# joaobuibergen/roms-trunk-mgh

Hardware: AMD Instinct MI355X
Metric: simulated-days/wall-sec (higher is better)
Workload: dtype f64; 1 GPU; BENCHMARK3 2048x256x30 NT=2 nonlinear 3-D step incl. 59 step2d calls, U3/C4 tracer advection, analytic atmospheric forcing, bulk fluxes + KPP + diagnostics every step; tiling=1x1, halo_transport=none, rccl_ranks=0, graph_exchanges=1, ndtfast=20, finite=True

## Files before the change

### roms_trunk_mgh_amd/csrc/k_diag.hip

```cpp
#include "roms_dev.h"

int roms_entry_check(const char *name);

namespace {

__global__ void __launch_bounds__(BLK_X *BLK_Y)
k_wvelocity(const RomsDev *__restrict__ c, int ninp)
{
  DEV_PROLOGUE(c)
  const Blk XB = xcd_block();
  const int i = b.Istr + XB.x * BLK_X + threadIdx.x;
  const int j = b.Jstr + XB.y * BLK_Y + threadIdx.y;
  if (i > b.Iend || j > b.Jend) return;
  const long a = I2(i, j);
  const gcd_t u = (gcd_t)(c->F.u + (long)(ninp - 1) * n3r), v = (gcd_t)(c->F.v + (long)(ninp - 1) * n3r);
  const gcd_t z_r = (gcd_t)c->F.z_r, z_w = (gcd_t)c->F.z_w, W = (gcd_t)c->F.W;
  const gd_t wvel = (gd_t)c->F.wvel;
  const gcd_t pm = (gcd_t)c->F.pm, pn = (gcd_t)c->F.pn;
  const double pmw = pm[a - 1] + pm[a], pme = pm[a] + pm[a + 1];
  const double pns = pn[a - ni] + pn[a], pnn = pn[a] + pn[a + ni];
  const double pmn = pm[a] * pn[a];
  auto vert_at = [&](int k) {
    const long q = a + (long)(k - 1) * nij;
    const double zr0 = z_r[q];
// ... 99 lines not shown
    }
#pragma unroll
    for (int q = 0; q < DIAG_UNR; q++) {
      const int j = j0 + q;
      if (j <= b.Jend) {
        vol = vol + tv[q];
        pe = pe + tp[q];
        ke = ke + tk[q];
        if (tc[q] > mC) {
          const long a = I2(i, j);
          mC = tc[q]; mCu = w.Cu[a]; mCv = w.Cv[a]; mCw = w.Cw[a]; mj = j; mk = (int)w.Ck[a];
        }
        mspd = fmax(mspd, ts[q]);
        mrho = fmax(mrho, tr[q]);
      }
    }
  }
  R[R_VOL * nI + o] = vol; R[R_PE * nI + o] = pe; R[R_KE * nI + o] = ke;
  R[R_C * nI + o] = mC; R[R_CU * nI + o] = mCu; R[R_CV * nI + o] = mCv; R[R_CW * nI + o] = mCw;
  R[R_CJ * nI + o] = (double)mj; R[R_CK * nI + o] = (double)mk;
  R[R_SPD * nI + o] = mspd; R[R_RHO * nI + o] = mrho;
}

#define DIAG_CH 512
struct DiagBest { double C, Cu, Cv, Cw; int i, j, k; };
__device__ __forceinline__ bool diag_better(const DiagBest &x, const DiagBest &y)
{
  if (x.C != y.C) return x.C > y.C;
  if (!(x.C > 0.0)) return false;
  if (x.j != y.j) return x.j < y.j;
  if (x.k != y.k) return x.k > y.k;
  return x.i < y.i;
}
__global__ void __launch_bounds__(256)
k_diag_final(const RomsDev *__restrict__ c, const double *__restrict__ R, double *__restrict__ out)
{
  const roms_bounds_t &b = c->b;
  __shared__ double sR[3 * DIAG_CH];
  __shared__ DiagBest sB[256];
  __shared__ double sSpd[256], sRho[256];
  const int nI = b.Iend - b.Istr + 1;
  const int tid = threadIdx.x;
  DiagBest best{0.0, 0.0, 0.0, 0.0, 0, 0, 0};
  double mspd = 0.0, mrho = -1.0E+37;
  for (int o = tid; o < nI; o += 256) {
    DiagBest x{R[R_C * nI + o], R[R_CU * nI + o], R[R_CV * nI + o], R[R_CW * nI + o], b.Istr + o,
               (int)R[R_CJ * nI + o], (int)R[R_CK * nI + o]};
    if (diag_better(x, best)) best = x;
    mspd = fmax(mspd, R[R_SPD * nI + o]);
    mrho = fmax(mrho, R[R_RHO * nI + o]);
  }
  sB[tid] = best; sSpd[tid] = mspd; sRho[tid] = mrho;
  __syncthreads();
  for (int st = 128; st >= 1; st >>= 1) {
    if (tid < st) {
      if (diag_better(sB[tid + st], sB[tid])) sB[tid] = sB[tid + st];
      sSpd[tid] = fmax(sSpd[tid], sSpd[tid + st]);
      sRho[tid] = fmax(sRho[tid], sRho[tid + st]);
    }
    __syncthreads();
  }
  double acc = 0.0;
  const int chain = tid / 64;
  for (int o0 = 0; o0 < nI; o0 += DIAG_CH) {
    const int n = (nI - o0 < DIAG_CH) ? nI - o0 : DIAG_CH;
    __syncthreads();
    for (int e = tid; e < 3 * DIAG_CH; e += 256) {
      const int r = e / DIAG_CH, q = e % DIAG_CH;
      sR[e] = (q < n) ? R[(r == 0 ? R_VOL : (r == 1 ? R_PE : R_KE)) * nI + o0 + q] : 0.0;
    }
    __syncthreads();
    if ((tid & 63) == 0 && chain < 3) {
      const double *src = sR + chain * DIAG_CH;
      for (int q0 = 0; q0 < n; q0 += 16) {
        double t[16];
#pragma unroll
        for (int q = 0; q < 16; q++) t[q] = src[q0 + q < DIAG_CH ? q0 + q : DIAG_CH - 1];
#pragma unroll
        for (int q = 0; q < 16; q++)
          if (q0 + q < n) acc = acc + t[q];
      }
    }
  }
  if (tid == 0) out[0] = acc;
  if (tid == 64) out[2] = acc;
  if (tid == 128) out[1] = acc;
  if (tid == 192) {
    out[3] = sSpd[0]; out[4] = sRho[0];
    out[5] = sB[0].C; out[6] = sB[0].Cu; out[7] = sB[0].Cv; out[8] = sB[0].Cw;
    out[9] = (double)sB[0].i; out[10] = (double)sB[0].j; out[11] = (double)sB[0].k;
  }
}

double *g_diag_dev = nullptr;
double *g_diag_rows = nullptr;
long g_diag_rows_n = 0;

}

void diag_release()
{
  if (g_diag_dev) (void)hipFree(g_diag_dev);
  if (g_diag_rows) (void)hipFree(g_diag_rows);
  g_diag_dev = g_diag_rows = nullptr;
  g_diag_rows_n = 0;
}

extern "C" int roms_hip_wvelocity(const roms_step_idx_t *s)
{
  int rc = roms_entry_check("roms_hip_wvelocity");
  if (rc) return rc;
  if ((rc = check_lbc())) return rc;
  const roms_bounds_t &b = g_ctx.b;
// ... 45 lines not shown
```

### roms_trunk_mgh_amd/csrc/k_pre_step3d.hip

```cpp
#include "roms_dev.h"
#include "advect.h"

int roms_entry_check(const char *name);

namespace {

template <int HADV, int VADV, int NMAX, bool MASK, bool DIA = false, bool DEFER = false, int NTR = 1>
__global__ void __launch_bounds__(BLK_X *BLK_Y)
k_pre_t(const RomsDev *__restrict__ c, int nstp, int nnew, int first_step, int itrc0, int ntr)
{
  static_assert(NTR == 1 || (VADV != ADV_A4 && VADV != ADV_SPLINES && !DIA), "pairs: no whole-column arrays, no diagnostics");
  static_assert(!(DIA && DEFER), "diagnostics keep the two kernels");
  DEV_PROLOGUE(c)
  const TileCol tc = tile_column(b, itrc0, ntr);
  if (!tc.valid) return;
  const int i = tc.i, j = tc.j;
  const int itrc1 = itrc0 + NTR * (tc.itrc - itrc0);
  const roms_params_t &p = c->p;
  const double dt = p.dt;
  const ColFields f = column_fields(c);
  const long c0 = I2(i, j);
  const Walls wl = column_walls(c, i, j);
  const double Gamma = (HADV == ADV_MPDATA) ? 0.5 : 1.0 / 6.0;
  const double GammaV = (VADV == ADV_MPDATA) ? 0.5 : 1.0 / 6.0;
// ... 110 lines not shown
    const double bstr = (comp == 0 ? c->F.bustr : c->F.bvstr)[c0];
    const double sstr = (comp == 0 ? c->F.sustr : c->F.svstr)[c0];
    const double cq = dt * 0.25;
    const double DC0 = cq * (pm[c0] + pm[c0 - off]) * (pn[c0] + pn[c0 - off]);
    double FCprev = dt * bstr;
    double vk = vel[c0];
    double zsum_k = 0.0;
    (void)zsum_k;
    for (int k = 1; k <= N; k++) {
      const long ck = c0 + (long)(k - 1) * nij;
      double FCk, vk1 = 0.0;
      if (k == N) FCk = dt * sstr;
      else {
        vk1 = vel[ck + nij];
        if (cff3 != 0.0) {
          const double cz = 1.0 / (z_r[ck + nij] + z_r[ck + nij - off] - z_r[ck] - z_r[ck - off]);
          FCk = cff3 * cz * (vk1 - vk) * (Akv[ck + nij] + Akv[ck + nij - off]);
        } else {
          FCk = 0.0;
        }
      }
      const double hzs = Hz[ck] + Hz[ck - off];
      const double d = FCk - FCprev;
      double out;
      if (stage == 0) {
        const double a = vk * 0.5 * hzs;
        out = a + d;
      } else if (stage == 1) {
        const double a = vk * 0.5 * hzs;
        const double c3 = 0.5 * DC0;
        out = a - c3 * r2[ck + nij] + d;
      } else {
        const double a = vk * 0.5 * hzs;
        out = a + DC0 * ((5.0 / 12.0) * r1[ck + nij] - (16.0 / 12.0) * r2[ck + nij]) + d;
      }
      vnew[ck] = out;
      FCprev = FCk;
      vk = vk1;
    }
  }
}

template <int HADV, int VADV, bool DEFER, int NTR>
int launch_pre_t_n(const roms_step_idx_t *s, int itrc0, int nthr)
{
  typedef void (*PreKernel)(const RomsDev *, int, int, int, int, int);
  const roms_bounds_t &b = g_ctx.b;
  const dim3 grid = grid_tile_tracer(b.Iend - b.Istr + 1, b.Jend - b.Jstr + 1, nthr);
  const int first = s->iic == s->ntfirst;
  if (b.N > ROMS_MAXN) return roms_fail("roms_hip_pre_step3d", "N > 64 not instantiated");
  PreKernel kernel;
  if constexpr (NTR == 2) {
    kernel = k_pre_t<HADV, VADV, ROMS_MAXN, false, false, DEFER, 2>;
    if constexpr (HADV != ADV_MPDATA)
      if (g_ctx.p.masking) kernel = k_pre_t<HADV, VADV, ROMS_MAXN, true, false, DEFER, 2>;
  } else {
    kernel = kernel_for_n(b.N, [](auto nm) -> PreKernel { return k_pre_t<HADV, VADV, nm.value, false, false, DEFER>; });
    if constexpr (HADV != ADV_MPDATA)
      if (g_ctx.p.masking)
// ... 59 lines not shown
      }
      if (rc) return rc;
      it += n;
    }
  }
  const long n3r = (long)(b.UBi - b.LBi + 1) * (b.UBj - b.LBj + 1) * b.N;
  for (int it = 1; it <= b.NT; it++)
    if ((rc = bc_t3d(3, it, s->nstp))) return rc;
  halo_batch_begin();
  for (int it = 1; it <= b.NT; it++) halo_exchange3d(GT_R, b.N, g_ctx.dev[FID_t] + (2L + 3L * (it - 1)) * n3r);
  return halo_batch_end();
}

static int pre_step3d_uv(const roms_step_idx_t *s)
{
  const roms_bounds_t &b = g_ctx.b;
  const int stage = (s->iic == s->ntfirst) ? 0 : (s->iic == s->ntfirst + 1 ? 1 : 2);
  hipLaunchKernelGGL(k_pre_uv, grid2d(b.Iend - b.Istr + 1, b.Jend - b.Jstr + 1), block2d(), 0, g_ctx.stream,
                     g_ctx.devc, s->nstp, s->nnew, s->nrhs, stage);
  KERNEL_CHECK("k_pre_uv");
  return 0;
}

int pre_step3d_entry(const roms_step_idx_t *s, bool fused)
{
  int rc = roms_entry_check("roms_hip_pre_step3d");
  if (rc) return rc;
  if ((rc = check_lbc())) return rc;
  if (g_ctx.b.N < 4) return roms_fail("roms_hip_pre_step3d", "needs N >= 4 levels (the vertical stencils of the column read k-1 .. k+2)");
  if ((rc = dia_check("roms_hip_pre_step3d"))) return rc;
  ScopedTimer tm("pre_step3d");
  if ((rc = pre_step3d_uv(s))) return rc;
  return pre_step3d_tracers(s, fused);
}

extern "C" int roms_hip_pre_step3d(const roms_step_idx_t *s) { return pre_step3d_entry(s, false); }
```

### roms_trunk_mgh_amd/csrc/k_prsgrd.hip

```cpp
#include "roms_dev.h"

int roms_entry_check(const char *name);

namespace {

__device__ __forceinline__ double harm(double a, double bq, double eps)
{
  const double cff = 2.0 * a * bq;
  return (cff > eps) ? cff / (a + bq) : 0.0;
}
__device__ __forceinline__ double harm_inv(double a, double bq, double eps)
{
  const double cff = 2.0 * a * bq;
  if (cff > eps) { const double cff1 = 1.0 / (a + bq); return cff * cff1; }
  return 0.0;
}

__global__ void __launch_bounds__(BLK_X *BLK_Y)
k_prsgrd_P(const RomsDev *__restrict__ c, double *__restrict__ P)
{
  DEV_PROLOGUE(c)
  const Blk XB = xcd_block();
  const int i = b.IstrU - 1 + XB.x * BLK_X + threadIdx.x;
  const int j = b.JstrV - 1 + XB.y * BLK_Y + threadIdx.y;
  if (i > b.Iend || j > b.Jend) return;
  const gcd_t rho = (gcd_t)(c->F.rho);
  const gcd_t z_r = (gcd_t)(c->F.z_r);
  const double eps = 1.0E-10, OneFifth = 0.2, OneTwelfth = 1.0 / 12.0;
  const double g = c->p.g, GRho = g / c->p.rho0, HalfGRho = 0.5 * GRho;
  const long c0 = I2(i, j);
  double rho_k1 = rho[c0 + (long)(N - 1) * nij];
  double zr_k1 = z_r[c0 + (long)(N - 1) * nij];
  double rho_k = rho[c0 + (long)(N - 2) * nij];
  double zr_k = z_r[c0 + (long)(N - 2) * nij];
  const double zwN = GF(z_w)[c0 + (long)N * nij];
  {
    const double cff1 = 1.0 / (zr_k1 - zr_k);
    const double cff2 = 0.5 * (rho_k1 - rho_k) * (zwN - zr_k1) * cff1;
    if (c->p.atm_press)
      P[c0 + (long)(N - 1) * nij] = g * zwN + (100.0 / c->p.rho0) * (GF(Pair)[c0] - 1013.25) + GRho * (rho_k1 + cff2) * (zwN - zr_k1);
    else
      P[c0 + (long)(N - 1) * nij] = g * zwN + GRho * (rho_k1 + cff2) * (zwN - zr_k1);
  }
  double Pk1 = P[c0 + (long)(N - 1) * nij];
  double rawR_k = rho_k1 - rho_k, rawZ_k = zr_k1 - zr_k;
  double dR_k1 = harm(rawR_k, rawR_k, eps);
  double dZ_k1 = 2.0 * rawZ_k * rawZ_k / (rawZ_k + rawZ_k);
  for (int k = N - 1; k >= 1; k--) {
    double rawR_km1, rawZ_km1, rho_km1 = 0.0, zr_km1 = 0.0;
    if (k >= 2) {
      rho_km1 = rho[c0 + (long)(k - 2) * nij];
      zr_km1 = z_r[c0 + (long)(k - 2) * nij];
      rawR_km1 = rho_k - rho_km1;
      rawZ_km1 = zr_k - zr_km1;
    } else { rawR_km1 = rawR_k; rawZ_km1 = rawZ_k; }
    const double dR_k = harm(rawR_k, rawR_km1, eps);
    const double dZ_k = 2.0 * rawZ_k * rawZ_km1 / (rawZ_k + rawZ_km1);
    const double Pk = Pk1 +
        HalfGRho * ((rho_k1 + rho_k) * (zr_k1 - zr_k) -
                    OneFifth *
                    ((dR_k1 - dR_k) * (zr_k1 - zr_k - OneTwelfth * (dZ_k1 + dZ_k)) -
                     (dZ_k1 - dZ_k) * (rho_k1 - rho_k - OneTwelfth * (dR_k1 + dR_k))));
    P[c0 + (long)(k - 1) * nij] = Pk;
    Pk1 = Pk;
    rho_k1 = rho_k; zr_k1 = zr_k; rho_k = rho_km1; zr_k = zr_km1;
    rawR_k = rawR_km1; rawZ_k = rawZ_km1;
    dR_k1 = dR_k; dZ_k1 = dZ_k;
  }
}

__global__ void __launch_bounds__(BLK_X *BLK_Y)
k_prsgrd_uv(const RomsDev *__restrict__ c, const double *__restrict__ P, int nrhs)
{
  DEV_PROLOGUE(c)
  const Blk XB = xcd_block();
  const int i = b.Istr + XB.x * BLK_X + threadIdx.x;
  const int j = b.Jstr + XB.y * BLK_Y + threadIdx.y;
  const int k = XB.z + 1;
  if (i > b.Iend || j > b.Jend) return;
  const gcd_t rho = (gcd_t)(c->F.rho);
  const gcd_t z_r = (gcd_t)(c->F.z_r);
  const gcd_t Hz = (gcd_t)(c->F.Hz);
  const double eps = 1.0E-10, OneFifth = 0.2, OneTwelfth = 1.0 / 12.0;
  const double HalfGRho = 0.5 * (c->p.g / c->p.rho0);
  const bool masking = c->p.masking != 0;
  const long ck = I3(i, j, k);
  const double r0 = rho[ck], z0 = z_r[ck], hz0 = Hz[ck], P0 = P[ck];
  if (i >= b.IstrU) {
    const double rm2 = rho[ck - 2], rm1 = rho[ck - 1], rp1 = rho[ck + 1];
    const double zm2 = z_r[ck - 2], zm1 = z_r[ck - 1], zp1 = z_r[ck + 1];
    double aux_m1 = zm1 - zm2, aux_0 = z0 - zm1, aux_p1 = zp1 - z0;
    double FC_m1 = rm1 - rm2, FC_0 = r0 - rm1, FC_p1 = rp1 - r0;
    if (masking) {
      const gcd_t um = (gcd_t)c->F.umask;
      const long a2 = I2(i, j);
      const double m_m1 = um[a2 - 1], m_0 = um[a2], m_p1 = um[a2 + 1];
      aux_m1 = aux_m1 * m_m1; aux_0 = aux_0 * m_0; aux_p1 = aux_p1 * m_p1;
      FC_m1 = FC_m1 * m_m1; FC_0 = FC_0 * m_0; FC_p1 = FC_p1 * m_p1;
    }
    const double dZx0 = harm_inv(aux_0, aux_p1, eps), dZxm = harm_inv(aux_m1, aux_0, eps);
    const double dRx0 = harm_inv(FC_0, FC_p1, eps), dRxm = harm_inv(FC_m1, FC_0, eps);
    const gd_t ru = (gd_t)(c->F.ru + (long)(nrhs - 1) * n3w);
    double r = GF(on_u)[I2(i, j)] * 0.5 * (hz0 + Hz[ck - 1]) *
        (P[ck - 1] - P0 -
         HalfGRho * ((r0 + rm1) * (z0 - zm1) -
                     OneFifth * ((dRx0 - dRxm) * (z0 - zm1 - OneTwelfth * (dZx0 + dZxm)) -
                                 (dZx0 - dZxm) * (r0 - rm1 - OneTwelfth * (dRx0 + dRxm)))));
    if (c->p.wet_dry) r = r * GF(umask_wet)[I2(i, j)];
    ru[I3W(i, j, k)] = r;
  }
  if (j >= b.JstrV) {
    const double rm1 = rho[ck - ni], rp1 = rho[ck + ni];
    const double zm1 = z_r[ck - ni], zp1 = z_r[ck + ni];
    const double rm2 = rho[ck - 2 * ni], zm2 = z_r[ck - 2 * ni];
    double aux_m1 = zm1 - zm2, aux_0 = z0 - zm1, aux_p1 = zp1 - z0;
    double FC_m1 = rm1 - rm2, FC_0 = r0 - rm1, FC_p1 = rp1 - r0;
    if (masking) {
      const gcd_t vm = (gcd_t)c->F.vmask;
      const long a2 = I2(i, j);
      const double m_m1 = vm[a2 - ni], m_0 = vm[a2], m_p1 = vm[a2 + ni];
      aux_m1 = aux_m1 * m_m1; aux_0 = aux_0 * m_0; aux_p1 = aux_p1 * m_p1;
      FC_m1 = FC_m1 * m_m1; FC_0 = FC_0 * m_0; FC_p1 = FC_p1 * m_p1;
    }
    const double dZx0 = harm_inv(aux_0, aux_p1, eps), dZxm = harm_inv(aux_m1, aux_0, eps);
    const double dRx0 = harm_inv(FC_0, FC_p1, eps), dRxm = harm_inv(FC_m1, FC_0, eps);
    const gd_t rv = (gd_t)(c->F.rv + (long)(nrhs - 1) * n3w);
    double r = GF(om_v)[I2(i, j)] * 0.5 * (hz0 + Hz[ck - ni]) *
        (P[ck - ni] - P0 -
         HalfGRho * ((r0 + rm1) * (z0 - zm1) -
                     OneFifth * ((dRx0 - dRxm) * (z0 - zm1 - OneTwelfth * (dZx0 + dZxm)) -
                                 (dZx0 - dZxm) * (r0 - rm1 - OneTwelfth * (dRx0 + dRxm)))));
    if (c->p.wet_dry) r = r * GF(vmask_wet)[I2(i, j)];
    rv[I3W(i, j, k)] = r;
  }
}

template <bool WJ>
__global__ void __launch_bounds__(BLK_X *BLK_Y) k_prsgrd31(const RomsDev *__restrict__ c, int nrhs)
{
  DEV_PROLOGUE(c)
  const Blk XB = xcd_block();
  const int i = b.Istr + XB.x * BLK_X + threadIdx.x, j = b.Jstr + XB.y * BLK_Y + threadIdx.y;
  if (i > b.Iend || j > b.Jend) return;
  const bool do_u = i >= b.IstrU, do_v = j >= b.JstrV;
  const gcd_t rho = (gcd_t)(c->F.rho), z_r = (gcd_t)(c->F.z_r), Hz = (gcd_t)(c->F.Hz);
  const gd_t ru = (gd_t)(c->F.ru + (long)(nrhs - 1) * n3w), rv = (gd_t)(c->F.rv + (long)(nrhs - 1) * n3w);
  const double g = c->p.g, rho0 = c->p.rho0;
  const double fac1 = 0.5 * g / rho0, fac2 = 1000.0 * g / rho0, fac3 = 0.25 * g / rho0;
  const long a = I2(i, j), aw = do_u ? a - 1 : a, as = do_v ? a - ni : a;
  const double onu = GF(on_u)[a], omv = GF(om_v)[a];
  const bool wet = c->p.wet_dry != 0;
  const double uw = wet ? (double)GF(umask_wet)[a] : 1.0, vw = wet ? (double)GF(vmask_wet)[a] : 1.0;
  long q = a + (long)(N - 1) * nij, qw = aw + (long)(N - 1) * nij, qs = as + (long)(N - 1) * nij;
  double r1 = rho[q], z1 = z_r[q], r1w = rho[qw], z1w = z_r[qw], r1s = rho[qs], z1s = z_r[qs];
  const gcd_t zw = (gcd_t)(c->F.z_w);
  const double zw0 = zw[a + (long)N * nij], zww = zw[aw + (long)N * nij], zws = zw[as + (long)N * nij];
// ... 70 lines not shown
    const double h0 = Hz[q], hw = Hz[qw], hs = Hz[qs];
    const double P0m = P0 + h0 * rho[q], Pwm = Pw + hw * rho[qw], Psm = Ps + hs * rho[qs];
    const double FX0 = 0.5 * h0 * (P0 + P0m);
    if (do_u) {
      const double FXw = 0.5 * hw * (Pw + Pwm);
      const double dh = zw[q] - zw[qw];
      const double FCm = 0.5 * dh * (P0m + Pwm);
      ru[I3W(i, j, k)] = (cff * (hw + h0) * dzx + cff1 * (FXw - FX0 + FCx - FCm)) * onu;
      FCx = FCm;
    }
    if (do_v) {
      const double FXs = 0.5 * hs * (Ps + Psm);
      const double dh = zw[q] - zw[qs];
      const double FCm = 0.5 * dh * (P0m + Psm);
      rv[I3W(i, j, k)] = (cff * (hs + h0) * dze + cff1 * (FXs - FX0 + FCe - FCm)) * omv;
      FCe = FCm;
    }
    P0 = P0m; Pw = Pwm; Ps = Psm;
  }
}

}

extern "C" int roms_hip_prsgrd(const roms_step_idx_t *s)
{
  int rc = roms_entry_check("roms_hip_prsgrd");
  if (rc) return rc;
  if ((rc = check_lbc())) return rc;
  ScopedTimer tm("prsgrd");
  const roms_bounds_t &b = g_ctx.b;
  if (g_ctx.p.pgf == PGF_PJ_GRADP) {
    if (g_ctx.p.wet_dry) return roms_fail("roms_hip_prsgrd", "PJ_GRADP with WET_DRY does not exist in the reference");
    hipLaunchKernelGGL(k_prsgrd40, grid2d(b.Iend - b.Istr + 1, b.Jend - b.Jstr + 1), block2d(), 0, g_ctx.stream,
                       g_ctx.devc, s->nrhs);
    KERNEL_CHECK("k_prsgrd40");
    return 0;
  }
  if (g_ctx.p.pgf != PGF_DJ_GRADPS) {
    if (g_ctx.p.pgf != PGF_STANDARD && g_ctx.p.pgf != PGF_WJ_GRADP)
      return roms_fail("roms_hip_prsgrd", "unknown pressure-gradient algorithm (enum roms_pgf)");
    const dim3 grid = grid2d(b.Iend - b.Istr + 1, b.Jend - b.Jstr + 1);
    if (g_ctx.p.pgf == PGF_WJ_GRADP)
      hipLaunchKernelGGL(k_prsgrd31<true>, grid, block2d(), 0, g_ctx.stream, g_ctx.devc, s->nrhs);
    else
      hipLaunchKernelGGL(k_prsgrd31<false>, grid, block2d(), 0, g_ctx.stream, g_ctx.devc, s->nrhs);
    KERNEL_CHECK("k_prsgrd31");
    return 0;
  }
  if (b.N < 3) return roms_fail("roms_hip_prsgrd", "N < 3");
  double *P = g_ctx.hostc.ws3[0];
  hipLaunchKernelGGL(k_prsgrd_P, grid2d(b.Iend - (b.IstrU - 1) + 1, b.Jend - (b.JstrV - 1) + 1), block2d(), 0,
                     g_ctx.stream, g_ctx.devc, P);
  KERNEL_CHECK("k_prsgrd_P");
  dim3 grid = grid2d(b.Iend - b.Istr + 1, b.Jend - b.Jstr + 1);
  grid.z = b.N;
  hipLaunchKernelGGL(k_prsgrd_uv, grid, block2d(), 0, g_ctx.stream, g_ctx.devc, (const double *)P, s->nrhs);
  KERNEL_CHECK("k_prsgrd_uv");
  return 0;
}
```

### roms_trunk_mgh_amd/csrc/k_rhs3d.hip

```cpp
#include "roms_dev.h"

namespace {

#define Gadv (-0.25)

struct T3 {
  const double *u, *v, *Hu, *Hv, *Hz;
  int i0, j0;
  int Istr, Iend, Jstr, Jend;
  bool s_edge, n_edge, w_edge, e_edge;
  __device__ __forceinline__ int at(int i, int j) const { return (i - i0) + (j - j0) * TP; }
};

__device__ __forceinline__ int ex_uxx(const T3 &L, int i) {
  if (L.w_edge && i == L.Istr) return L.Istr + 1;
  if (L.e_edge && i == L.Iend + 1) return L.Iend;
  return i;
}
__device__ __forceinline__ int ey_uee(const T3 &L, int j) {
  if (L.s_edge && j == L.Jstr - 1) return L.Jstr;
  if (L.n_edge && j == L.Jend + 1) return L.Jend;
  return j;
}
__device__ __forceinline__ int ex_vxx(const T3 &L, int i) {
// ... 390 lines not shown
                      : hadv == ROMS_UVH_C4 ? (spl ? k_rhs3d_lds<ROMS_UVH_C4, ROMS_UVV_SPLINES> : k_rhs3d_lds<ROMS_UVH_C4, ROMS_UVV_C4>)
                                            : (spl ? k_rhs3d_lds<ROMS_UVH_U3, ROMS_UVV_SPLINES> : k_rhs3d_lds<ROMS_UVH_U3, ROMS_UVV_C4W>);
  hipLaunchKernelGGL(kernel, grid2d(b.Iend - b.Istr + 1, b.Jend - b.Jstr + 1), block2d(), 0, g_ctx.stream,
                     g_ctx.devc, s->nrhs);
  KERNEL_CHECK("k_rhs3d_lds");
  if (spl) {
    const dim3 grid((unsigned)((b.Iend - b.Istr + BLK_X) / BLK_X), (unsigned)(b.Jend - b.Jstr + 1), 1), block(BLK_X, 1, 1);
    if (b.N <= 16) hipLaunchKernelGGL(k_rhs3d_vspline<16>, grid, block, 0, g_ctx.stream, g_ctx.devc, s->nrhs);
    else if (b.N <= 32) hipLaunchKernelGGL(k_rhs3d_vspline<32>, grid, block, 0, g_ctx.stream, g_ctx.devc, s->nrhs);
    else if (b.N <= 48) hipLaunchKernelGGL(k_rhs3d_vspline<48>, grid, block, 0, g_ctx.stream, g_ctx.devc, s->nrhs);
    else hipLaunchKernelGGL(k_rhs3d_vspline<64>, grid, block, 0, g_ctx.stream, g_ctx.devc, s->nrhs);
    KERNEL_CHECK("k_rhs3d_vspline");
  }
  return 0;
}

static bool rhs3d_fuses_tstart(const roms_step_idx_t *s)
{
  const roms_params_t &p = g_ctx.p;
  return p.ts_dif2 && (p.mix_geo_ts || p.mix_iso_ts) && !p.ts_mix_stability && p.lambda == 1.0 && !dia_on() &&
         s->nrhs == s->nstp;
}

int roms_uv_mix_check(const char *where);

extern "C" int roms_hip_rhs3d(const roms_step_idx_t *s)
{
  int rc = roms_entry_check("roms_hip_rhs3d");
  if (rc) return rc;
  if ((rc = roms_uv_adv_check("roms_hip_rhs3d"))) return rc;
  if ((rc = roms_uv_mix_check("roms_hip_rhs3d"))) return rc;
  const bool fused = rhs3d_fuses_tstart(s);
  if ((rc = pre_step3d_entry(s, fused))) return rc;
  if ((rc = roms_hip_prsgrd(s))) return rc;
  if (g_ctx.p.ts_dif2 && (rc = t3dmix2_entry(s, fused))) return rc;
  if (g_ctx.p.ts_dif4 && (rc = roms_hip_t3dmix4(s))) return rc;
  if ((rc = roms_hip_rhs3d_tile(s))) return rc;
  if (g_ctx.p.uv_vis2 && (rc = roms_hip_uv3dmix2(s))) return rc;
  if (g_ctx.p.uv_vis4 && (rc = roms_hip_uv3dmix4(s))) return rc;
  return 0;
}
```

### roms_trunk_mgh_amd/csrc/roms_dev.h

```cpp
#pragma once
#include <hip/hip_runtime.h>
#include <cstdio>
#include <cstring>
#include <string>
#include "roms_hip.h"

#define ROMS_NWS3 10

struct RomsSrc {
  int n;
  int ltr[ROMS_MAXNT];
  const int *I, *J, *D;
  const double *Qbar;
  const double *Qsrc;
  const double *Tsrc;
  const int *umap, *vmap;
  const int *wmap;
  const int *cells;
  int ncell;
  double *save;
};

struct RomsClima {
  int m2, m3, nt;
// ... 132 lines not shown
  if ((nbx & 7) == 0) {
    const int L = r.x + nbx * (r.y + nby * r.z);
    const int xcd = L & 7, q = L >> 3, w = nbx >> 3;
    r.z = q % nz;
    const int t = q / nz;
    r.x = xcd * w + t % w;
    r.y = t / w;
  }
  return r;
}
#endif

#define DEV_PROLOGUE(c)                                                        \
  const roms_bounds_t &b = (c)->b;                                             \
  const int LBi = b.LBi, LBj = b.LBj;                                          \
  const int N = b.N;                                                           \
  const long ni = b.UBi - b.LBi + 1, nj = b.UBj - b.LBj + 1, nij = ni * nj;    \
  const long n3r = nij * N, n3w = nij * (N + 1);                               \
  (void)nj; (void)n3r; (void)n3w;

typedef const double __attribute__((address_space(1))) *gcd_t;
typedef double __attribute__((address_space(1))) *gd_t;
#define GF(name) ((gd_t)c->F.name)

#define ROMS_MASKW(name)                                                                                  \
  __device__ __forceinline__ double name##w(const RomsDev *__restrict__ c, long q)                       \
  {                                                                                                       \
    double m = ((gcd_t)c->F.name)[q];                                                                     \
    if (c->p.wet_dry) m = m * ((gcd_t)c->F.name##_wet)[q];                                                \
    return m;                                                                                             \
  }
ROMS_MASKW(rmask)
ROMS_MASKW(umask)
ROMS_MASKW(vmask)
ROMS_MASKW(pmask)
#undef ROMS_MASKW
__device__ __forceinline__ double wet_factor(double mask_wet, double vel)
{
  const double cff5 = fabs(fabs(mask_wet) - 1.0);
  const double cff6 = 0.5 + copysign(0.5, vel) * mask_wet;
  return 0.5 * mask_wet * cff5 + cff6 * (1.0 - cff5);
}

__device__ __forceinline__ bool src_cell_any(const RomsDev *__restrict__ c, long c0, long ni)
{
  return (c->src.umap[c0] | c->src.umap[c0 + 1] | c->src.vmap[c0] | c->src.vmap[c0 + ni] | c->src.wmap[c0]) != 0;
// ... 109 lines not shown
void floats_release();
void tides_release();
int guarded_alloc(double **user, double **base, long n);
void guarded_free(double **user, double **base);
void dia_release();
bool dia_on();
int dia_check(const char *where);
int dia_rate(int nnew);
int dia_arrays(const char *name[4], const double *base[4], long count[4]);
int bc_zeta(int kout, const roms_step_idx_t *s);
int bc_u2d(int kout, const roms_step_idx_t *s);
int bc_v2d(int kout, const roms_step_idx_t *s);
int bc_u3d(int nout, int nstp);
int bc_v3d(int nout, int nstp);
int bc_t3d(int nout, int itrc, int nstp);
bool lbc2d_all_closed();
int lbc_code(const roms_params_t &p, int sd, int v);
int bc_w3d(double *A);
int bc_generic(int gtype_var, int lbv, double *A, int nk);
void snapshot_release();
void snapshot_forget(int field_id);
void diag_release();
int check_lbc();
int pre_step3d_entry(const roms_step_idx_t *s, bool fused);
int t3dmix2_entry(const roms_step_idx_t *s, bool fused);
int roms_rowm_prepare();
void roms_rowm_invalidate();
bool roms_rowm_is_table_field(int id);
void roms_rowm_release();
void step2d_graphs_release();
```

Baseline: 0.2445 simulated-days/s.

## Fuse prsgrd pressure integration and gradient kernels, fold uv start, parallelize diag reduction

The two-pass prsgrd32 (pressure column kernel writing a 3-D P buffer, then a per-level gradient kernel) becomes one column kernel. It integrates P downward for its own points plus a one-point ring, exchanges neighbour P through a double-buffered shared plane, and writes ru/rv directly. With the DJ gradient scheme and lambda 1, it also computes the u/v time-start update that pre_step3d used to do, and that pass is skipped. Separately, the final diagnostic reduction now sums with all 64 lanes of three waves and uses a fourth wave with shuffles for the max/argmax reductions. The fusion removes the global P array round-trip and one kernel, but makes the kernel a serial loop over levels with a block barrier per level and extra ring work.

```diff
diff --git a/roms_trunk_mgh_amd/csrc/k_diag.hip b/roms_trunk_mgh_amd/csrc/k_diag.hip
--- a/roms_trunk_mgh_amd/csrc/k_diag.hip
+++ b/roms_trunk_mgh_amd/csrc/k_diag.hip
@@ -145,7 +145,8 @@
   R[R_SPD * nI + o] = mspd; R[R_RHO * nI + o] = mrho;
 }
 
-#define DIAG_CH 512
+#define DIAG_RUN 32
+#define DIAG_CH (64 * DIAG_RUN)
 struct DiagBest { double C, Cu, Cv, Cw; int i, j, k; };
 __device__ __forceinline__ bool diag_better(const DiagBest &x, const DiagBest &y)
 {
@@ -159,59 +160,74 @@
 k_diag_final(const RomsDev *__restrict__ c, const double *__restrict__ R, double *__restrict__ out)
 {
   const roms_bounds_t &b = c->b;
-  __shared__ double sR[3 * DIAG_CH];
-  __shared__ DiagBest sB[256];
-  __shared__ double sSpd[256], sRho[256];
+  __shared__ double sR[3][DIAG_CH];
   const int nI = b.Iend - b.Istr + 1;
-  const int tid = threadIdx.x;
-  DiagBest best{0.0, 0.0, 0.0, 0.0, 0, 0, 0};
-  double mspd = 0.0, mrho = -1.0E+37;
-  for (int o = tid; o < nI; o += 256) {
-    DiagBest x{R[R_C * nI + o], R[R_CU * nI + o], R[R_CV * nI + o], R[R_CW * nI + o], b.Istr + o,
-               (int)R[R_CJ * nI + o], (int)R[R_CK * nI + o]};
-    if (diag_better(x, best)) best = x;
-    mspd = fmax(mspd, R[R_SPD * nI + o]);
-    mrho = fmax(mrho, R[R_RHO * nI + o]);
-  }
-  sB[tid] = best; sSpd[tid] = mspd; sRho[tid] = mrho;
-  __syncthreads();
-  for (int st = 128; st >= 1; st >>= 1) {
-    if (tid < st) {
-      if (diag_better(sB[tid + st], sB[tid])) sB[tid] = sB[tid + st];
-      sSpd[tid] = fmax(sSpd[tid], sSpd[tid + st]);
-      sRho[tid] = fmax(sRho[tid], sRho[tid + st]);
-    }
-    __syncthreads();
-  }
+  const int lane = threadIdx.x & 63, wave = threadIdx.x >> 6;
+  const int row = wave < 3 ? wave : 0;
+  const double *src = R + (long)(row == 0 ? R_VOL : (row == 1 ? R_PE : R_KE)) * nI;
   double acc = 0.0;
-  const int chain = tid / 64;
   for (int o0 = 0; o0 < nI; o0 += DIAG_CH) {
     const int n = (nI - o0 < DIAG_CH) ? nI - o0 : DIAG_CH;
+    if (o0 > 0) __syncthreads();
+    if (wave < 3) {
+      double v[DIAG_RUN];
+#pragma unroll
+      for (int q = 0; q < DIAG_RUN; q++) {
+        const int e = q * 64 + lane;
+        v[q] = src[o0 + (e < n ? e : n - 1)];
+      }
+#pragma unroll
+      for (int q = 0; q < DIAG_RUN; q++) sR[row][q * 64 + lane] = v[q];
+    }
     __syncthreads();
-    for (int e = tid; e < 3 * DIAG_CH; e += 256) {
-      const int r = e / DIAG_CH, q = e % DIAG_CH;
-      sR[e] = (q < n) ? R[(r == 0 ? R_VOL : (r == 1 ? R_PE : R_KE)) * nI + o0 + q] : 0.0;
-    }
-    __syncthreads();
-    if ((tid & 63) == 0 && chain < 3) {
-      const double *src = sR + chain * DIAG_CH;
-      for (int q0 = 0; q0 < n; q0 += 16) {
-        double t[16];
-#pragma unroll
-        for (int q = 0; q < 16; q++) t[q] = src[q0 + q < DIAG_CH ? q0 + q : DIAG_CH - 1];
-#pragma unroll
-        for (int q = 0; q < 16; q++)
-          if (q0 + q < n) acc = acc + t[q];
-      }
-    }
-  }
-  if (tid == 0) out[0] = acc;
-  if (tid == 64) out[2] = acc;
-  if (tid == 128) out[1] = acc;
-  if (tid == 192) {
-    out[3] = sSpd[0]; out[4] = sRho[0];
-    out[5] = sB[0].C; out[6] = sB[0].Cu; out[7] = sB[0].Cv; out[8] = sB[0].Cw;
-    out[9] = (double)sB[0].i; out[10] = (double)sB[0].j; out[11] = (double)sB[0].k;
+    if (wave < 3) {
+      const double *sv = sR[row];
+      int e = 0;
+      for (; e + 64 <= n; e += 64) {
+        double t[64];
+#pragma unroll
+        for (int q = 0; q < 64; q++) t[q] = sv[e + q];
+#pragma unroll
+        for (int q = 0; q < 64; q++) acc = acc + t[q];
+      }
+      for (; e < n; e++) acc = acc + sv[e];
+    }
+  }
+  if (wave < 3 && lane == 0) out[row == 0 ? 0 : (row == 1 ? 2 : 1)] = acc;
+  if (wave == 3) {
+    DiagBest best{0.0, 0.0, 0.0, 0.0, 0, 0, 0};
+    double mspd = 0.0, mrho = -1.0E+37;
+    for (int o0 = lane; o0 < nI; o0 += 64 * 8) {
+      double t[8][8];
+#pragma unroll
+      for (int q = 0; q < 8; q++) {
+        const int o = (o0 + 64 * q < nI) ? o0 + 64 * q : nI - 1;
+        t[q][0] = R[R_C * nI + o]; t[q][1] = R[R_CU * nI + o]; t[q][2] = R[R_CV * nI + o]; t[q][3] = R[R_CW * nI + o];
+        t[q][4] = R[R_CJ * nI + o]; t[q][5] = R[R_CK * nI + o]; t[q][6] = R[R_SPD * nI + o]; t[q][7] = R[R_RHO * nI + o];
+      }
+#pragma unroll
+      for (int q = 0; q < 8; q++) {
+        const int o = o0 + 64 * q;
+        if (o < nI) {
+          const DiagBest x{t[q][0], t[q][1], t[q][2], t[q][3], b.Istr + o, (int)t[q][4], (int)t[q][5]};
+          if (diag_better(x, best)) best = x;
+          mspd = fmax(mspd, t[q][6]);
+          mrho = fmax(mrho, t[q][7]);
+        }
+      }
+    }
+    for (int m = 32; m >= 1; m >>= 1) {
+      const DiagBest y{__shfl_xor(best.C, m), __shfl_xor(best.Cu, m), __shfl_xor(best.Cv, m), __shfl_xor(best.Cw, m),
+                       __shfl_xor(best.i, m), __shfl_xor(best.j, m), __shfl_xor(best.k, m)};
+      if (diag_better(y, best)) best = y;
+      mspd = fmax(mspd, __shfl_xor(mspd, m));
+      mrho = fmax(mrho, __shfl_xor(mrho, m));
+    }
+    if (lane == 0) {
+      out[3] = mspd; out[4] = mrho;
+      out[5] = best.C; out[6] = best.Cu; out[7] = best.Cv; out[8] = best.Cw;
+      out[9] = (double)best.i; out[10] = (double)best.j; out[11] = (double)best.k;
+    }
   }
 }
 
diff --git a/roms_trunk_mgh_amd/csrc/k_pre_step3d.hip b/roms_trunk_mgh_amd/csrc/k_pre_step3d.hip
--- a/roms_trunk_mgh_amd/csrc/k_pre_step3d.hip
+++ b/roms_trunk_mgh_amd/csrc/k_pre_step3d.hip
@@ -156,19 +156,7 @@
       }
       const double hzs = Hz[ck] + Hz[ck - off];
       const double d = FCk - FCprev;
-      double out;
-      if (stage == 0) {
-        const double a = vk * 0.5 * hzs;
-        out = a + d;
-      } else if (stage == 1) {
-        const double a = vk * 0.5 * hzs;
-        const double c3 = 0.5 * DC0;
-        out = a - c3 * r2[ck + nij] + d;
-      } else {
-        const double a = vk * 0.5 * hzs;
-        out = a + DC0 * ((5.0 / 12.0) * r1[ck + nij] - (16.0 / 12.0) * r2[ck + nij]) + d;
-      }
-      vnew[ck] = out;
+      vnew[ck] = uv_start(stage, vk, hzs, DC0, r1, r2, ck + nij, d);
       FCprev = FCk;
       vk = vk1;
     }
@@ -274,7 +262,7 @@
   return 0;
 }
 
-int pre_step3d_entry(const roms_step_idx_t *s, bool fused)
+int pre_step3d_entry(const roms_step_idx_t *s, bool fused, bool uvstart)
 {
   int rc = roms_entry_check("roms_hip_pre_step3d");
   if (rc) return rc;
@@ -282,8 +270,8 @@
   if (g_ctx.b.N < 4) return roms_fail("roms_hip_pre_step3d", "needs N >= 4 levels (the vertical stencils of the column read k-1 .. k+2)");
   if ((rc = dia_check("roms_hip_pre_step3d"))) return rc;
   ScopedTimer tm("pre_step3d");
-  if ((rc = pre_step3d_uv(s))) return rc;
+  if (!uvstart && (rc = pre_step3d_uv(s))) return rc;
   return pre_step3d_tracers(s, fused);
 }
 
-extern "C" int roms_hip_pre_step3d(const roms_step_idx_t *s) { return pre_step3d_entry(s, false); }
+extern "C" int roms_hip_pre_step3d(const roms_step_idx_t *s) { return pre_step3d_entry(s, false, false); }
diff --git a/roms_trunk_mgh_amd/csrc/k_prsgrd.hip b/roms_trunk_mgh_amd/csrc/k_prsgrd.hip
--- a/roms_trunk_mgh_amd/csrc/k_prsgrd.hip
+++ b/roms_trunk_mgh_amd/csrc/k_prsgrd.hip
@@ -16,122 +16,171 @@
   return 0.0;
 }
 
-__global__ void __launch_bounds__(BLK_X *BLK_Y)
-k_prsgrd_P(const RomsDev *__restrict__ c, double *__restrict__ P)
+struct PCol { double r_up, z_up, r_dn, z_dn, P_up, dR_up, dZ_up; };
+
+__device__ __forceinline__ double prsgrd32_P_top(const RomsDev *__restrict__ c, gcd_t rho, gcd_t z_r, long c0, int N,
+                                                 long nij, PCol &q)
+{
+  const double eps = 1.0E-10;
+  const double g = c->p.g, GRho = g / c->p.rho0;
+  const double rho_k1 = rho[c0 + (long)(N - 1) * nij];
+  const double zr_k1 = z_r[c0 + (long)(N - 1) * nij];
+  const double rho_k = rho[c0 + (long)(N - 2) * nij];
+  const double zr_k = z_r[c0 + (long)(N - 2) * nij];
+  const double zwN = GF(z_w)[c0 + (long)N * nij];
+  const double cff1 = 1.0 / (zr_k1 - zr_k);
+  const double cff2 = 0.5 * (rho_k1 - rho_k) * (zwN - zr_k1) * cff1;
+  double P;
+  if (c->p.atm_press)
+    P = g * zwN + (100.0 / c->p.rho0) * (GF(Pair)[c0] - 1013.25) + GRho * (rho_k1 + cff2) * (zwN - zr_k1);
+  else
+    P = g * zwN + GRho * (rho_k1 + cff2) * (zwN - zr_k1);
+  const double rawR_k = rho_k1 - rho_k, rawZ_k = zr_k1 - zr_k;
+  q.r_up = rho_k1; q.z_up = zr_k1; q.r_dn = rho_k; q.z_dn = zr_k;
+  q.dR_up = harm(rawR_k, rawR_k, eps);
+  q.dZ_up = 2.0 * rawZ_k * rawZ_k / (rawZ_k + rawZ_k);
+  q.P_up = P;
+  return P;
+}
+
+__device__ __forceinline__ double prsgrd32_P_down(gcd_t rho, gcd_t z_r, long c0, int k, long nij, double HalfGRho, PCol &q)
+{
+  const double eps = 1.0E-10, OneFifth = 0.2, OneTwelfth = 1.0 / 12.0;
+  const double rho_k1 = q.r_up, zr_k1 = q.z_up, rho_k = q.r_dn, zr_k = q.z_dn;
+  const double rawR_k = rho_k1 - rho_k, rawZ_k = zr_k1 - zr_k, dR_k1 = q.dR_up, dZ_k1 = q.dZ_up;
+  double rawR_km1, rawZ_km1, rho_km1 = 0.0, zr_km1 = 0.0;
+  if (k >= 2) {
+    rho_km1 = rho[c0 + (long)(k - 2) * nij];
+    zr_km1 = z_r[c0 + (long)(k - 2) * nij];
+    rawR_km1 = rho_k - rho_km1;
+    rawZ_km1 = zr_k - zr_km1;
+  } else { rawR_km1 = rawR_k; rawZ_km1 = rawZ_k; }
+  const double dR_k = harm(rawR_k, rawR_km1, eps);
+  const double dZ_k = 2.0 * rawZ_k * rawZ_km1 / (rawZ_k + rawZ_km1);
+  const double Pk = q.P_up +
+      HalfGRho * ((rho_k1 + rho_k) * (zr_k1 - zr_k) -
+                  OneFifth *
+                  ((dR_k1 - dR_k) * (zr_k1 - zr_k - OneTwelfth * (dZ_k1 + dZ_k)) -
+                   (dZ_k1 - dZ_k) * (rho_k1 - rho_k - OneTwelfth * (dR_k1 + dR_k))));
+  q.P_up = Pk;
+  q.r_up = rho_k; q.z_up = zr_k; q.r_dn = rho_km1; q.z_dn = zr_km1;
+  q.dR_up = dR_k; q.dZ_up = dZ_k;
+  return Pk;
+}
+
+__device__ __forceinline__ double prsgrd32_jac(gcd_t rho, gcd_t z_r, long ck, long off, double r0, double z0,
+                                               bool masking, gcd_t mask, long a2, double HalfGRho)
+{
+  const double eps = 1.0E-10, OneFifth = 0.2, OneTwelfth = 1.0 / 12.0;
+  const double rm2 = rho[ck - 2 * off], rm1 = rho[ck - off], rp1 = rho[ck + off];
+  const double zm2 = z_r[ck - 2 * off], zm1 = z_r[ck - off], zp1 = z_r[ck + off];
+  double aux_m1 = zm1 - zm2, aux_0 = z0 - zm1, aux_p1 = zp1 - z0;
+  double FC_m1 = rm1 - rm2, FC_0 = r0 - rm1, FC_p1 = rp1 - r0;
+  if (masking) {
+    const double m_m1 = mask[a2 - off], m_0 = mask[a2], m_p1 = mask[a2 + off];
+    aux_m1 = aux_m1 * m_m1; aux_0 = aux_0 * m_0; aux_p1 = aux_p1 * m_p1;
+    FC_m1 = FC_m1 * m_m1; FC_0 = FC_0 * m_0; FC_p1 = FC_p1 * m_p1;
+  }
+  const double dZx0 = harm_inv(aux_0, aux_p1, eps), dZxm = harm_inv(aux_m1, aux_0, eps);
+  const double dRx0 = harm_inv(FC_0, FC_p1, eps), dRxm = harm_inv(FC_m1, FC_0, eps);
+  return HalfGRho * ((r0 + rm1) * (z0 - zm1) -
+                     OneFifth * ((dRx0 - dRxm) * (z0 - zm1 - OneTwelfth * (dZx0 + dZxm)) -
+                                 (dZx0 - dZxm) * (r0 - rm1 - OneTwelfth * (dRx0 + dRxm))));
+}
+
+template <bool UVSTART>
+__global__ void __launch_bounds__(BLK_X *BLK_Y) __attribute__((amdgpu_waves_per_eu(4)))
+k_prsgrd32(const RomsDev *__restrict__ c, int nrhs, int nstp, int nnew, int stage)
 {
   DEV_PROLOGUE(c)
   const Blk XB = xcd_block();
-  const int i = b.IstrU - 1 + XB.x * BLK_X + threadIdx.x;
-  const int j = b.JstrV - 1 + XB.y * BLK_Y + threadIdx.y;
-  if (i > b.Iend || j > b.Jend) return;
-  const gcd_t rho = (gcd_t)(c->F.rho);
-  const gcd_t z_r = (gcd_t)(c->F.z_r);
-  const double eps = 1.0E-10, OneFifth = 0.2, OneTwelfth = 1.0 / 12.0;
-  const double g = c->p.g, GRho = g / c->p.rho0, HalfGRho = 0.5 * GRho;
-  const long c0 = I2(i, j);
-  double rho_k1 = rho[c0 + (long)(N - 1) * nij];
-  double zr_k1 = z_r[c0 + (long)(N - 1) * nij];
-  double rho_k = rho[c0 + (long)(N - 2) * nij];
-  double zr_k = z_r[c0 + (long)(N - 2) * nij];
-  const double zwN = GF(z_w)[c0 + (long)N * nij];
-  {
-    const double cff1 = 1.0 / (zr_k1 - zr_k);
-    const double cff2 = 0.5 * (rho_k1 - rho_k) * (zwN - zr_k1) * cff1;
-    if (c->p.atm_press)
-      P[c0 + (long)(N - 1) * nij] = g * zwN + (100.0 / c->p.rho0) * (GF(Pair)[c0] - 1013.25) + GRho * (rho_k1 + cff2) * (zwN - zr_k1);
-    else
-      P[c0 + (long)(N - 1) * nij] = g * zwN + GRho * (rho_k1 + cff2) * (zwN - zr_k1);
-  }
-  double Pk1 = P[c0 + (long)(N - 1) * nij];
-  double rawR_k = rho_k1 - rho_k, rawZ_k = zr_k1 - zr_k;
-  double dR_k1 = harm(rawR_k, rawR_k, eps);
-  double dZ_k1 = 2.0 * rawZ_k * rawZ_k / (rawZ_k + rawZ_k);
-  for (int k = N - 1; k >= 1; k--) {
-    double rawR_km1, rawZ_km1, rho_km1 = 0.0, zr_km1 = 0.0;
-    if (k >= 2) {
-      rho_km1 = rho[c0 + (long)(k - 2) * nij];
-      zr_km1 = z_r[c0 + (long)(k - 2) * nij];
-      rawR_km1 = rho_k - rho_km1;
-      rawZ_km1 = zr_k - zr_km1;
-    } else { rawR_km1 = rawR_k; rawZ_km1 = rawZ_k; }
-    const double dR_k = harm(rawR_k, rawR_km1, eps);
-    const double dZ_k = 2.0 * rawZ_k * rawZ_km1 / (rawZ_k + rawZ_km1);
-    const double Pk = Pk1 +
-        HalfGRho * ((rho_k1 + rho_k) * (zr_k1 - zr_k) -
-                    OneFifth *
-                    ((dR_k1 - dR_k) * (zr_k1 - zr_k - OneTwelfth * (dZ_k1 + dZ_k)) -
-                     (dZ_k1 - dZ_k) * (rho_k1 - rho_k - OneTwelfth * (dR_k1 + dR_k))));
-    P[c0 + (long)(k - 1) * nij] = Pk;
-    Pk1 = Pk;
-    rho_k1 = rho_k; zr_k1 = zr_k; rho_k = rho_km1; zr_k = zr_km1;
-    rawR_k = rawR_km1; rawZ_k = rawZ_km1;
-    dR_k1 = dR_k; dZ_k1 = dZ_k;
-  }
-}
-
-__global__ void __launch_bounds__(BLK_X *BLK_Y)
-k_prsgrd_uv(const RomsDev *__restrict__ c, const double *__restrict__ P, int nrhs)
-{
-  DEV_PROLOGUE(c)
-  const Blk XB = xcd_block();
-  const int i = b.Istr + XB.x * BLK_X + threadIdx.x;
-  const int j = b.Jstr + XB.y * BLK_Y + threadIdx.y;
-  const int k = XB.z + 1;
-  if (i > b.Iend || j > b.Jend) return;
+  constexpr int PW = BLK_X + 1, PLANE = PW * (BLK_Y + 1);
+  __shared__ double sP[2 * PLANE];
+  const int tx = threadIdx.x, ty = threadIdx.y, tid = ty * BLK_X + tx;
+  const int i0 = b.Istr + XB.x * BLK_X, j0 = b.Jstr + XB.y * BLK_Y;
+  const int i = i0 + tx, j = j0 + ty;
+  const bool own = i <= b.Iend && j <= b.Jend;
+  const bool do_u = own && i >= b.IstrU, do_v = own && j >= b.JstrV;
+  const int rli = tid < PW ? tid : 0, rlj = tid < PW ? 0 : tid - BLK_X;
+  const int ri = i0 - 1 + rli, rj = j0 - 1 + rlj;
+  const bool ring = tid < PW + BLK_Y && ri >= b.IstrU - 1 && ri <= b.Iend && rj >= b.JstrV - 1 && rj <= b.Jend;
+  const int lo = (ty + 1) * PW + tx + 1, lr = rlj * PW + rli;
   const gcd_t rho = (gcd_t)(c->F.rho);
   const gcd_t z_r = (gcd_t)(c->F.z_r);
   const gcd_t Hz = (gcd_t)(c->F.Hz);
-  const double eps = 1.0E-10, OneFifth = 0.2, OneTwelfth = 1.0 / 12.0;
   const double HalfGRho = 0.5 * (c->p.g / c->p.rho0);
-  const bool masking = c->p.masking != 0;
-  const long ck = I3(i, j, k);
-  const double r0 = rho[ck], z0 = z_r[ck], hz0 = Hz[ck], P0 = P[ck];
-  if (i >= b.IstrU) {
-    const double rm2 = rho[ck - 2], rm1 = rho[ck - 1], rp1 = rho[ck + 1];
-    const double zm2 = z_r[ck - 2], zm1 = z_r[ck - 1], zp1 = z_r[ck + 1];
-    double aux_m1 = zm1 - zm2, aux_0 = z0 - zm1, aux_p1 = zp1 - z0;
-    double FC_m1 = rm1 - rm2, FC_0 = r0 - rm1, FC_p1 = rp1 - r0;
-    if (masking) {
-      const gcd_t um = (gcd_t)c->F.umask;
-      const long a2 = I2(i, j);
-      const double m_m1 = um[a2 - 1], m_0 = um[a2], m_p1 = um[a2 + 1];
-      aux_m1 = aux_m1 * m_m1; aux_0 = aux_0 * m_0; aux_p1 = aux_p1 * m_p1;
-      FC_m1 = FC_m1 * m_m1; FC_0 = FC_0 * m_0; FC_p1 = FC_p1 * m_p1;
-    }
-    const double dZx0 = harm_inv(aux_0, aux_p1, eps), dZxm = harm_inv(aux_m1, aux_0, eps);
-    const double dRx0 = harm_inv(FC_0, FC_p1, eps), dRxm = harm_inv(FC_m1, FC_0, eps);
-    const gd_t ru = (gd_t)(c->F.ru + (long)(nrhs - 1) * n3w);
-    double r = GF(on_u)[I2(i, j)] * 0.5 * (hz0 + Hz[ck - 1]) *
-        (P[ck - 1] - P0 -
-         HalfGRho * ((r0 + rm1) * (z0 - zm1) -
-                     OneFifth * ((dRx0 - dRxm) * (z0 - zm1 - OneTwelfth * (dZx0 + dZxm)) -
-                                 (dZx0 - dZxm) * (r0 - rm1 - OneTwelfth * (dRx0 + dRxm)))));
-    if (c->p.wet_dry) r = r * GF(umask_wet)[I2(i, j)];
-    ru[I3W(i, j, k)] = r;
-  }
-  if (j >= b.JstrV) {
-    const double rm1 = rho[ck - ni], rp1 = rho[ck + ni];
-    const double zm1 = z_r[ck - ni], zp1 = z_r[ck + ni];
-    const double rm2 = rho[ck - 2 * ni], zm2 = z_r[ck - 2 * ni];
-    double aux_m1 = zm1 - zm2, aux_0 = z0 - zm1, aux_p1 = zp1 - z0;
-    double FC_m1 = rm1 - rm2, FC_0 = r0 - rm1, FC_p1 = rp1 - r0;
-    if (masking) {
-      const gcd_t vm = (gcd_t)c->F.vmask;
-      const long a2 = I2(i, j);
-      const double m_m1 = vm[a2 - ni], m_0 = vm[a2], m_p1 = vm[a2 + ni];
-      aux_m1 = aux_m1 * m_m1; aux_0 = aux_0 * m_0; aux_p1 = aux_p1 * m_p1;
-      FC_m1 = FC_m1 * m_m1; FC_0 = FC_0 * m_0; FC_p1 = FC_p1 * m_p1;
-    }
-    const double dZx0 = harm_inv(aux_0, aux_p1, eps), dZxm = harm_inv(aux_m1, aux_0, eps);
-    const double dRx0 = harm_inv(FC_0, FC_p1, eps), dRxm = harm_inv(FC_m1, FC_0, eps);
-    const gd_t rv = (gd_t)(c->F.rv + (long)(nrhs - 1) * n3w);
-    double r = GF(om_v)[I2(i, j)] * 0.5 * (hz0 + Hz[ck - ni]) *
-        (P[ck - ni] - P0 -
-         HalfGRho * ((r0 + rm1) * (z0 - zm1) -
-                     OneFifth * ((dRx0 - dRxm) * (z0 - zm1 - OneTwelfth * (dZx0 + dZxm)) -
-                                 (dZx0 - dZxm) * (r0 - rm1 - OneTwelfth * (dRx0 + dRxm)))));
-    if (c->p.wet_dry) r = r * GF(vmask_wet)[I2(i, j)];
-    rv[I3W(i, j, k)] = r;
+  const bool masking = c->p.masking != 0, wet = c->p.wet_dry != 0;
+  const long a2 = I2(own ? i : b.Iend, own ? j : b.Jend);
+  const long ar = I2(ring ? ri : b.Iend, ring ? rj : b.Jend);
+  const gd_t ru = (gd_t)(c->F.ru + (long)(nrhs - 1) * n3w), rv = (gd_t)(c->F.rv + (long)(nrhs - 1) * n3w);
+  double onu = 0.0, omv = 0.0, uwet = 1.0, vwet = 1.0;
+  if (do_u) {
+    onu = GF(on_u)[a2];
+    if (wet) uwet = GF(umask_wet)[a2];
+  }
+  if (do_v) {
+    omv = GF(om_v)[a2];
+    if (wet) vwet = GF(vmask_wet)[a2];
+  }
+  const double dt = c->p.dt;
+  const gcd_t us = (gcd_t)(c->F.u + (long)(nstp - 1) * n3r), vs = (gcd_t)(c->F.v + (long)(nstp - 1) * n3r);
+  const gd_t un = (gd_t)(c->F.u + (long)(nnew - 1) * n3r), vn = (gd_t)(c->F.v + (long)(nnew - 1) * n3r);
+  const gcd_t ru2 = (gcd_t)(c->F.ru + (long)(3 - nrhs - 1) * n3w), rv2 = (gcd_t)(c->F.rv + (long)(3 - nrhs - 1) * n3w);
+  double DCu = 0.0, DCv = 0.0;
+  if constexpr (UVSTART) {
+    const gcd_t pm = (gcd_t)(c->F.pm), pn = (gcd_t)(c->F.pn);
+    const double cq = dt * 0.25;
+    if (do_u) DCu = cq * (pm[a2] + pm[a2 - 1]) * (pn[a2] + pn[a2 - 1]);
+    if (do_v) DCv = cq * (pm[a2] + pm[a2 - ni]) * (pn[a2] + pn[a2 - ni]);
+  }
+
+  PCol qo{}, qr{};
+  double P0 = 0.0, Pr = 0.0;
+  if (own) P0 = prsgrd32_P_top(c, rho, z_r, a2, N, nij, qo);
+  if (ring) Pr = prsgrd32_P_top(c, rho, z_r, ar, N, nij, qr);
+  for (int k = N; k >= 1; k--) {
+    if (k < N) {
+      if (own) P0 = prsgrd32_P_down(rho, z_r, a2, k, nij, HalfGRho, qo);
+      if (ring) Pr = prsgrd32_P_down(rho, z_r, ar, k, nij, HalfGRho, qr);
+    }
+    double *pl = sP + (k & 1) * PLANE;
+    if (own) pl[lo] = P0;
+    if (ring) pl[lr] = Pr;
+    const long ck = a2 + (long)(k - 1) * nij;
+    const double r0 = qo.r_up, z0 = qo.z_up;
+    double hz0 = 0.0, hsu = 0.0, hsv = 0.0, Ju = 0.0, Jv = 0.0, unew = 0.0, vnew = 0.0;
+    if (own) hz0 = Hz[ck];
+    if (do_u) {
+      hsu = hz0 + Hz[ck - 1];
+      Ju = prsgrd32_jac(rho, z_r, ck, 1, r0, z0, masking, (gcd_t)c->F.umask, a2, HalfGRho);
+    }
+    if (do_v) {
+      hsv = hz0 + Hz[ck - ni];
+      Jv = prsgrd32_jac(rho, z_r, ck, ni, r0, z0, masking, (gcd_t)c->F.vmask, a2, HalfGRho);
+    }
+    if constexpr (UVSTART) {
+      if (do_u) {
+        const double FCk = (k == N) ? dt * GF(sustr)[a2] : 0.0, FCprev = (k == 1) ? dt * GF(bustr)[a2] : 0.0;
+        unew = uv_start(stage, us[ck], hsu, DCu, (gcd_t)ru, ru2, ck + nij, FCk - FCprev);
+      }
+      if (do_v) {
+        const double FCk = (k == N) ? dt * GF(svstr)[a2] : 0.0, FCprev = (k == 1) ? dt * GF(bvstr)[a2] : 0.0;
+        vnew = uv_start(stage, vs[ck], hsv, DCv, (gcd_t)rv, rv2, ck + nij, FCk - FCprev);
+      }
+    }
+    __syncthreads();
+    if (do_u) {
+      double r = onu * 0.5 * hsu * (pl[lo - 1] - P0 - Ju);
+      if (wet) r = r * uwet;
+      if constexpr (UVSTART) un[ck] = unew;
+      ru[ck + nij] = r;
+    }
+    if (do_v) {
+      double r = omv * 0.5 * hsv * (pl[lo - PW] - P0 - Jv);
+      if (wet) r = r * vwet;
+      if constexpr (UVSTART) vn[ck] = vnew;
+      rv[ck + nij] = r;
+    }
   }
 }
 
@@ -248,7 +297,7 @@
 
 }
 
-extern "C" int roms_hip_prsgrd(const roms_step_idx_t *s)
+int prsgrd_entry(const roms_step_idx_t *s, bool uvstart)
 {
   int rc = roms_entry_check("roms_hip_prsgrd");
   if (rc) return rc;
@@ -273,14 +322,12 @@
     KERNEL_CHECK("k_prsgrd31");
     return 0;
   }
-  if (b.N < 3) return roms_fail("roms_hip_prsgrd", "N < 3");
-  double *P = g_ctx.hostc.ws3[0];
-  hipLaunchKernelGGL(k_prsgrd_P, grid2d(b.Iend - (b.IstrU - 1) + 1, b.Jend - (b.JstrV - 1) + 1), block2d(), 0,
-                     g_ctx.stream, g_ctx.devc, P);
-  KERNEL_CHECK("k_prsgrd_P");
-  dim3 grid = grid2d(b.Iend - b.Istr + 1, b.Jend - b.Jstr + 1);
-  grid.z = b.N;
-  hipLaunchKernelGGL(k_prsgrd_uv, grid, block2d(), 0, g_ctx.stream, g_ctx.devc, (const double *)P, s->nrhs);
-  KERNEL_CHECK("k_prsgrd_uv");
+  if (b.N < 2) return roms_fail("roms_hip_prsgrd", "N < 2");
+  const int stage = (s->iic == s->ntfirst) ? 0 : (s->iic == s->ntfirst + 1 ? 1 : 2);
+  hipLaunchKernelGGL(uvstart ? k_prsgrd32<true> : k_prsgrd32<false>, grid2d(b.Iend - b.Istr + 1, b.Jend - b.Jstr + 1),
+                     block2d(), 0, g_ctx.stream, g_ctx.devc, s->nrhs, s->nstp, s->nnew, stage);
+  KERNEL_CHECK("k_prsgrd32");
   return 0;
 }
+
+extern "C" int roms_hip_prsgrd(const roms_step_idx_t *s) { return prsgrd_entry(s, false); }
diff --git a/roms_trunk_mgh_amd/csrc/k_rhs3d.hip b/roms_trunk_mgh_amd/csrc/k_rhs3d.hip
--- a/roms_trunk_mgh_amd/csrc/k_rhs3d.hip
+++ b/roms_trunk_mgh_amd/csrc/k_rhs3d.hip
@@ -436,6 +436,13 @@
          s->nrhs == s->nstp;
 }
 
+static bool rhs3d_fuses_uvstart(const roms_step_idx_t *s)
+{
+  (void)s;
+  const roms_params_t &p = g_ctx.p;
+  return p.pgf == PGF_DJ_GRADPS && p.lambda == 1.0;
+}
+
 int roms_uv_mix_check(const char *where);
 
 extern "C" int roms_hip_rhs3d(const roms_step_idx_t *s)
@@ -445,8 +452,9 @@
   if ((rc = roms_uv_adv_check("roms_hip_rhs3d"))) return rc;
   if ((rc = roms_uv_mix_check("roms_hip_rhs3d"))) return rc;
   const bool fused = rhs3d_fuses_tstart(s);
-  if ((rc = pre_step3d_entry(s, fused))) return rc;
-  if ((rc = roms_hip_prsgrd(s))) return rc;
+  const bool uvstart = rhs3d_fuses_uvstart(s);
+  if ((rc = pre_step3d_entry(s, fused, uvstart))) return rc;
+  if ((rc = prsgrd_entry(s, uvstart))) return rc;
   if (g_ctx.p.ts_dif2 && (rc = t3dmix2_entry(s, fused))) return rc;
   if (g_ctx.p.ts_dif4 && (rc = roms_hip_t3dmix4(s))) return rc;
   if ((rc = roms_hip_rhs3d_tile(s))) return rc;
diff --git a/roms_trunk_mgh_amd/csrc/roms_dev.h b/roms_trunk_mgh_amd/csrc/roms_dev.h
--- a/roms_trunk_mgh_amd/csrc/roms_dev.h
+++ b/roms_trunk_mgh_amd/csrc/roms_dev.h
@@ -178,6 +178,23 @@
 typedef const double __attribute__((address_space(1))) *gcd_t;
 typedef double __attribute__((address_space(1))) *gd_t;
 #define GF(name) ((gd_t)c->F.name)
+
+__device__ __forceinline__ double uv_start(int stage, double vk, double hzs, double DC0, gcd_t r1, gcd_t r2, long q, double d)
+{
+  double out;
+  if (stage == 0) {
+    const double a = vk * 0.5 * hzs;
+    out = a + d;
+  } else if (stage == 1) {
+    const double a = vk * 0.5 * hzs;
+    const double c3 = 0.5 * DC0;
+    out = a - c3 * r2[q] + d;
+  } else {
+    const double a = vk * 0.5 * hzs;
+    out = a + DC0 * ((5.0 / 12.0) * r1[q] - (16.0 / 12.0) * r2[q]) + d;
+  }
+  return out;
+}
 
 #define ROMS_MASKW(name)                                                                                  \
   __device__ __forceinline__ double name##w(const RomsDev *__restrict__ c, long q)                       \
@@ -333,7 +350,8 @@
 void snapshot_forget(int field_id);
 void diag_release();
 int check_lbc();
-int pre_step3d_entry(const roms_step_idx_t *s, bool fused);
+int pre_step3d_entry(const roms_step_idx_t *s, bool fused, bool uvstart);
+int prsgrd_entry(const roms_step_idx_t *s, bool uvstart);
 int t3dmix2_entry(const roms_step_idx_t *s, bool fused);
 int roms_rowm_prepare();
 void roms_rowm_invalidate();
```

Result: faster. 0.2498 simulated-days/s (median of 6 runs) (+2.2%).
